# j-fu/ExtendableSparse.jl

Hardware: AMD Instinct MI355X
Metric: assembled+flushed nnz/sec and HBM GB/s %peak, 256³ 7-pt stencil, 1/2/4/8 GPU (higher is better)
Workload: dtype f64; 1 GPU; fdrand 256^3 Float64/Int64 fresh build: device COO append (the producer writes every update to its radix bucket) -> LDS bucket sort + ordered fold -> CSC (BASELINE.json configs[1]); n=256, appended_entries=200933376, final_nnz=117047296, partition=producer-side (append = partition), parallelism=1 GPU

## Files before the change

### extendablesparse.jl_amd/_lib.py

```python
import ctypes as C
import os

HERE = os.path.dirname(os.path.abspath(__file__))
SO = os.path.join(HERE, "libesparse_hip.so")

ESP_OK = 0
ESP_ERR_INVALID, ESP_ERR_BOUNDS, ESP_ERR_HIP, ESP_ERR_NOMEM = -1, -2, -3, -4
ESP_ERR_UNSUPPORTED, ESP_ERR_STATE, ESP_ERR_NODEVICE = -5, -6, -7
ESP_ERR_NOTPOSDEF = -8
ESP_SET, ESP_UPDATE, ESP_RAWUPDATE, ESP_COO = 0, 1, 2, 3
ESP_OP_ADD, ESP_OP_SUB = 0, 1
ESP_FLUSH_ROUTED, ESP_FLUSH_PLUS = 0, 1
ESP_PATH_NO_KEPT_STRUCTURE = 45
ESP_PRECON_JACOBI, ESP_PRECON_ILU0, ESP_PRECON_ILUAM, ESP_PRECON_BLOCK, ESP_PRECON_AMG = 0, 1, 2, 3, 4
ESP_PRECON_ILUK = 5
ESP_PRECON_COLORED = 6
ESP_PRECON_SPAI = 7
ESP_PRECON_ILUT = 8
ESP_PRECON_LU = 9
ESP_PRECON_CHOLESKY = 10
ESP_CHOL_STATS = 12
ESP_ILUT_WAVE_UPPER, ESP_ILUT_GROUP_UPPER, ESP_ILUT_STEPS_MAX, ESP_ILUT_STATS = 256, 4096, 16, 40
ESP_ILUK_WAVE_VISITS, ESP_ILUK_VISIT_MAX = 512, 8192
ESP_SPAI_WAVE_DOUBLES, ESP_SPAI_DENSE_MAX = 512, 12288
# ... 147 lines not shown
    "esp_transpose": (i32, [vp, vp, P(i64)]),
    "esp_debug_transpose_path": (i32, [vp, i32]),
    "esp_debug_last_transpose": (i32, [vp, P(i64)]),
    "esp_mul_transpose": (i32, [vp, vp, vp, i32]),
    "esp_issymmetric": (i32, [vp, P(i32)]),
    "esp_opnorm": (i32, [vp, f64, P(f64)]),
    "esp_norm": (i32, [vp, f64, P(f64)]),
    "esp_shard_counts": (i32, [vp, i32, vp]),
    "esp_shard_export": (i32, [vp, i32, vp, vp, vp]),
    "esp_shard_exchange_begin": (i32, [vp, i32, i32, i64, i64, P(vp), P(vp), vp]),
    "esp_shard_exchange_place": (i32, [vp, i64, vp, vp, i64]),
    "esp_shard_partition": (i32, [vp, i32, i32, i64, P(i32), P(vp), P(vp), P(vp), vp, P(i64)]),
    "esp_shard_assemble": (i32, [vp, vp, vp, vp, vp, P(i32)]),
    "esp_shard_plan": (i32, [vp, i32, i32, i64]),
    "esp_debug_last_shard_source": (i32, [vp, P(i32)]),
    "esp_debug_last_local_small": (i32, [vp, P(i32)]),
    "esp_debug_last_bucket_pairs": (i32, [vp, P(i32)]),
    "esp_debug_last_bucket_cut": (i32, [vp, P(i32), P(i32)]),
    "esp_debug_last_predicted": (i32, [vp, P(i32)]),
    "esp_debug_spoil_predicted": (i32, [vp]),
    "esp_debug_last_lazy_items": (i32, [vp, P(i32)]),
    "esp_debug_last_lazy_stencil": (i32, [vp, P(i32)]),
    "esp_debug_last_kept_structure": (i32, [vp, P(i32)]),
    "esp_debug_last_sum_join": (i32, [vp, P(i32)]),
    "esp_debug_last_sum_ms": (i32, [vp, P(C.c_double), P(C.c_double)]),
    "esp_debug_last_sum_batched": (i32, [vp, P(C.c_int32)]),
    "esp_debug_last_sum_plan_bits": (i32, [vp, P(i32), P(i32)]),
    "esp_debug_last_rebuild": (i32, [vp, P(i32)]),
    "esp_group_unique_id": (i32, [vp]),
    "esp_group_create": (i32, [vp, i32, i32, vp, P(vp)]),
    "esp_group_create_comm": (i32, [vp, i32, i32, vp, P(vp)]),
    "esp_group_destroy": (i32, [vp]),
    "esp_group_handle": (i32, [vp, P(vp)]),
    "esp_group_last_error": (C.c_char_p, [vp]),
    "esp_group_column_range": (i32, [vp, P(i64), P(i64)]),
    "esp_group_flush": (i32, [vp, i32, P(i64), P(i32)]),
    "esp_group_nnz": (i32, [vp, P(i64), P(i64)]),
    "esp_group_get_csc": (i32, [vp, vp, vp, vp]),
    "esp_group_last_exchange": (i32, [vp, P(i32), P(i64)]),
    "esp_debug_group_loopback": (i32, [vp, i32, P(i64)]),
    "esp_timing_enable": (i32, [vp, i32]),
    "esp_timing": (i32, [vp, P(esp_timing_t), i32]),
    "esp_debug_plan_cap": (i32, [vp, C.c_double]),
    "esp_debug_fail_next_bucket_stage": (i32, [vp]),
    "esp_debug_force_path": (i32, [vp, i32]),
    "esp_debug_last_run_order": (i32, [vp, P(i32)]),
# ... 49 lines not shown
```

### extendablesparse.jl_amd/csrc/flush.hip

```cpp
#include "internal.hpp"

bool esplocal::launch(const Variant &v, unsigned grid, hipStream_t stream, const Args &a) {
    if (v.pair) return launch_pair(v, grid, stream, a);
    if (v.g3) return launch_group3(v, grid, stream, a);
    if (v.grp) return v.shortg ? launch_group_short(v, grid, stream, a) : launch_group(v, grid, stream, a);
    if (v.pieces) return v.small_variant ? launch_pieces_small(v, grid, stream, a) : v.fresh ? launch_pieces_fresh(v, grid, stream, a) : launch_pieces_stored(v, grid, stream, a);
    return v.small_variant ? launch_small(v, grid, stream, a) : launch_regular(v, grid, stream, a);
}


int32_t finish_csc(esp_handle *h, i64 Z0, i64 Zn, const u64 *new_key, const double *new_val) {
    const i64 N1 = h->n + 1;
    u64 *colend = (u64 *)h->colend.p;
    i64 c0, ccnt;
    col_range(h, &c0, &ccnt);
    if (windowed(h)) h->tail_stale = h->wc1 < h->n;
    if (Z0 == 0) {
        Span sp(h, ESP_ST_COLPTR);
        sp.add(espscan::exclusive<u64, true>(h->stream, colend + c0, (u64 *)h->colptr.p + c0, ccnt, colend + N1, (u64)1));
        if (!windowed(h)) h->ones_pending = false;
        h->nnz = Zn;
        h->pattern_version++, h->values_version++;
        return ESP_OK;
    }
// ... 248 lines not shown
    return ESP_OK;
}

struct LocalTry {
    bool use_pred, want_wide, allow_g3;
    bool used_pair = false, used_g3 = false;
};

static int32_t launch_attempt(esp_handle *h, const Sorted &st, const LocalChoice &c, esplocal::Args &a, LocalTry &t) {
    Span sp(h, ESP_ST_LOCAL);
    const i64 max_grid = h->force_path == ESP_PATH_MANY_LAUNCHES ? 64 : esplocal::MAX_GRID;
    t.used_g3 = t.used_pair = false;
    if (c.pair_ok && !h->pair_off) {
        const int Sp = (c.S + 1) / 2;
        esplocal::Args ap = a;
        ap.S = Sp;
        ap.pair_buckets = c.S;
        ap.status = a.status + (c.S - Sp);
        esplocal::Variant var{true, false, false, true, c.pair_keys};
        var.pair = true;
        h->last_fold_update = c.pair_keys == 2 ? 1 : 0;
        const u64 out_cap = (u64)std::min(h->keys2.bytes / sizeof(i64), h->vals2.bytes / sizeof(double));
        const u64 *pred = (const u64 *)h->pred.tab.p;
        for (i64 first = 0; first < Sp; first += max_grid) {
            ap.first = first;
            const unsigned grid = (unsigned)std::min<i64>(max_grid, Sp - first);
            if (t.use_pred && st.stencil) {
                if (!esplocal::launch_pair_gen_predicted(var, grid, h->stream, ap, st.stencil->a, pred, out_cap, c.keep))
                    return ESP_RETRY_EXPANDED;
            } else if (!(t.use_pred ? esplocal::launch_pair_predicted(var, grid, h->stream, ap, pred, out_cap) : esplocal::launch(var, grid, h->stream, ap)))
                FAIL(h, ESP_ERR_STATE, "esp_flush: internal error (no pair kernel for this flush)");
        }
        t.used_pair = true;
        sp.add(1);
        return ESP_OK;
    }
    h->last_fold_update = (c.keys == 2 || c.keys == 3 || c.keys == 5 || c.keys == 7) ? 1 : 0;
    esplocal::Variant var{c.fresh, st.npieces > 0, c.big && !c.small_variant && !c.grp, c.small_variant, c.keys};
    var.shortg = c.grp && c.longest <= 32.0;
    var.grp = c.grp;
    var.g3 = t.allow_g3 && !h->g3_off && (c.g3_plain || (c.g3_k64 && !t.want_wide));
    var.g3k64 = var.g3 && c.g3_k64;
    if (var.g3k64) a.kind32 = (u32)c.kind_all;
    var.g3wide = var.g3 && t.want_wide;
    for (i64 first = 0; first < c.S; first += max_grid) {
        const unsigned grid = (unsigned)std::min<i64>(max_grid, c.S - first);
        a.first = first;
        t.used_g3 = var.g3;
        if (st.lazy) {
            if (!var.g3 || var.g3wide || !esplocal::launch_group3_items(*st.lazy, grid, h->stream, a)) return ESP_RETRY_EXPANDED;
        } else if (!esplocal::launch(var, grid, h->stream, a))
            FAIL(h, ESP_ERR_STATE, "esp_flush: internal error (no bucket kernel for this flush)");
    }
    sp.add(1);
    return ESP_OK;
// ... 87 lines not shown
    esplocal::Args a;
    fill_args(a, h, st, c, mode, lay);
    h->last_key_bytes = (st.p32_piece >= 0 || st.all32) ? 4 : st.key_bytes;
    const char *stamps_file = esp_exp_env("ESP_LOCAL_STAMPS");
    if (stamps_file) {
        CK(ensure(h, h->heads, sizeof(u64) * (size_t)c.S * 16));
        HIPCK(h, hipMemsetAsync(h->heads.p, 0, sizeof(u64) * (size_t)c.S * 16, h->stream));
        a.stamps = (unsigned long long *)h->heads.p;
    }
    LocalTry t{c.use_pred, c.want_wide, true};
    if (c.try_hits) {
        bool done = false;
        CK(try_hits_form(h, st, c, lay, a, t, Zn_out, &done));
        if (done) return ESP_OK;
    }
    CK(launch_attempt(h, st, c, a, t));
    CK(read_back(h, c, a));
    const bool pred_tried = t.use_pred && t.used_pair;
    if (pred_tried && (err_bits(h) & (esplocal::PRED_MISS | esplocal::PAIR_REFUSED))) {
        t.use_pred = false;
        h->pred.misses++;
        h->pred.last = 2;
        if (c.keep) h->last_kept = 2;
        drop_kept(h);
        CK(retry_attempt(h, st, c, lay, a, t));
    } else if (pred_tried) {
        h->pred.misses = 0;
        h->pred.last = 1;
    }
    if (t.used_pair && (err_bits(h) & esplocal::PAIR_REFUSED)) {
        h->pair_off = true;
        CK(retry_attempt(h, st, c, lay, a, t));
    }
    h->last_pair = t.used_pair ? 1 : 0;
    h->last_cl_bits = c.cl_bits;
    h->last_buckets = c.S;
    h->last_lazy_items = 0;
    h->last_sum_join = 0;
    if (st.lazy) {
        if (err_bits(h) & 8u) return ESP_RETRY_EXPANDED;
        h->last_lazy_items = 1;
    }
    if (t.used_g3 && !t.want_wide && h->force_path != ESP_PATH_NO_WIDE_GROUP3 && (err_bits(h) & (8u | 16u | 32u)) == (8u | 16u)) {
        t.want_wide = true;
        h->g3_wide = true;
        CK(retry_attempt(h, st, c, lay, a, t));
// ... 372 lines not shown
extern "C" int32_t esp_flush(esp_handle *h, int32_t mode, int64_t *new_nnz, int32_t *pattern_changed) {
    if (!h) return ESP_ERR_INVALID;
    if (mode != ESP_FLUSH_ROUTED && mode != ESP_FLUSH_PLUS) FAIL(h, ESP_ERR_INVALID, "esp_flush: mode");
    (void)hipSetDevice(h->device);
    if (pattern_changed) *pattern_changed = 0;
    i64 E = h->count;
    if (E == 0) {
        if (new_nnz) *new_nnz = h->nnz;
        return ESP_OK;
    }
    if (E >= 0xFFFFFFF0ll) FAIL(h, ESP_ERR_UNSUPPORTED, "esp_flush: %lld pending entries exceed the 2^32 limit of one flush", (long long)E);
    hipEvent_t fa = nullptr;
    if (h->timing) {
        fa = ev_get(h);
        (void)hipEventRecord(fa, h->stream);
    }
    i64 Zn = 0;
    h->last_rebuild = 0;
    h->last_pair = 0;
    h->pred.last = 0;
    h->kept.candidate = h->kept.valid;
    h->kept.valid = false;
    h->last_kept = 0;
    bool use_local = h->force_path != ESP_PATH_GENERAL;
    if (h->ones_pending && windowed(h)) CK(fix_tail(h));
    if (h->pre.valid) {
        const esp_handle::PrePart &pp = h->pre;
        const bool usable = use_local && !h->part_assembled && pp.mw_P == 0 && pp.E + pp.tail == E && pp.base == h->win_base &&
                            pp.span == h->win_span && pp.maxlen <= (i64)esplocal::CAP && pp.K - pp.pb <= esplocal::MAX_REM_BITS;
        if (!usable) CK(pending_materialize(h));
    }
    if (h->pre.valid && h->lazy.on &&
        (h->pre.tail != 0 || !use_local || windowed(h) || h->shard_user || h->part_assembled ||
         (h->nnz != 0 && !(h->seen_hits && !h->hits_off && mode == ESP_FLUSH_ROUTED))))
        CK(lazy_expand(h));
    if (h->pre.valid && h->lazyst.on &&
        (h->pre.tail != 0 || !use_local || windowed(h) || h->shard_user || h->part_assembled || h->nnz != 0))
        CK(lazy_expand(h));
    if (h->last_lazy_stencil == 1) h->last_lazy_stencil = 0;
    bool served = false, split = false, tail_direct = false;
    i64 Zsplit = 0;
    if (h->pre.valid && h->pre.tail > 0 && h->nnz > 0 && mode == ESP_FLUSH_ROUTED && h->force_path != ESP_PATH_BATCH_TAIL_ONE_FLUSH) {
        const esp_handle::PrePart pp = h->pre;
        Sorted st = pre_sorted(h, pp, false);
        st.expect_hits = 1;
        CK(ensure(h, h->keys2, sizeof(u64) * (size_t)E));
// ... 160 lines not shown
```

### extendablesparse.jl_amd/csrc/handle.hip

```cpp
#include "internal.hpp"

#include <pthread.h>
#include <sched.h>
#include <sys/mman.h>

#include <atomic>
#include <chrono>
#include <condition_variable>
#include <mutex>

thread_local std::string g_err;

int32_t ensure(esp_handle *h, DevBuf &b, size_t need, bool keep) {
    if (b.bytes >= need && b.p) return ESP_OK;
    if (h && (&b == &h->colptr || &b == &h->rowval || &b == &h->nzval)) drop_kept(h);
    size_t want = need;
    if (keep && b.bytes) want = std::max(need, b.bytes + b.bytes / 2);
    want = (want + 255) & ~(size_t)255;
    void *np = nullptr;
    if (!(keep && b.p && b.bytes)) {
        release(b);
        HIPCK(h, hipMalloc(&np, want));
        b.p = np;
        b.bytes = want;
// ... 199 lines not shown
    if (device < 0 || device >= ndev)
        FAIL((esp_handle *)nullptr, ESP_ERR_INVALID, "esp_create: device %d out of range (0..%d)", device, ndev - 1);
    const int rb = bits_for(m), cb = bits_for(n);
    if (rb + cb + ESP_TAG_BITS > 64)
        FAIL((esp_handle *)nullptr, ESP_ERR_UNSUPPORTED, "esp_create: %lld x %lld needs %d key bits (max 62)",
             (long long)m, (long long)n, rb + cb);
    esp_handle *h = new esp_handle();
    h->m = m;
    h->n = n;
    h->device = device;
    h->L = KeyLayout{rb, cb};
    h->win_base = 0;
    h->win_span = (u64)std::max<i64>(n, 1) << rb;
    h->wc0 = 0;
    h->wc1 = n;
    h->hint = capacity_hint > 0 ? capacity_hint : 0;
    memset(&h->acc, 0, sizeof h->acc);
    if (const char *e = getenv("ESP_DEBUG_FORCE_PATH")) h->force_path = atoi(e);
    if (hipSetDevice(device) != hipSuccess || hipStreamCreateWithFlags(&h->stream, hipStreamNonBlocking) != hipSuccess) {
        delete h;
        FAIL((esp_handle *)nullptr, ESP_ERR_HIP, "esp_create: cannot create a stream on device %d", device);
    }
    h->own_stream = true;
    if (hipHostMalloc((void **)&h->pin_scalar, 128, hipHostMallocDefault) != hipSuccess) {
        (void)hipStreamDestroy(h->stream);
        delete h;
        FAIL((esp_handle *)nullptr, ESP_ERR_NOMEM, "esp_create: pinned scalar allocation failed");
    }
    memset(h->pin_scalar, 0, 128);
    h->pin_words = h->pin_scalar + 8;
    if (hipHostGetDevicePointer((void **)&h->pin_words_dev, h->pin_words, 0) != hipSuccess || !h->pin_words_dev) {
        (void)hipHostFree(h->pin_scalar);
        (void)hipStreamDestroy(h->stream);
        delete h;
        FAIL((esp_handle *)nullptr, ESP_ERR_HIP, "esp_create: no device address for the pinned result words");
    }
    int32_t st = init_empty_csc(h);
    if (st == ESP_OK && capacity_hint > 0) {
        st = ensure(h, h->keys, sizeof(u64) * (size_t)capacity_hint);
        if (st == ESP_OK) st = ensure(h, h->vals, sizeof(double) * (size_t)capacity_hint);
        if (st == ESP_OK) h->cap = capacity_hint;
    }
    if (st != ESP_OK) {
        g_err = h->err;
        esp_destroy(h);
        return st;
// ... 1057 lines not shown
```

### extendablesparse.jl_amd/csrc/internal.hpp

```cpp
#pragma once
#include <stdio.h>
#include <stdlib.h>
#include <string.h>

#include <algorithm>
#include <functional>
#include <cmath>
#include <thread>

#include "common.hpp"
#include "fold.hpp"
#include "generators.hpp"
#include "femitems.hpp"
#include "elements.hpp"
#include "local_args.hpp"
#include "merge.hpp"
#include "radix.hpp"
#include "runpart.hpp"
#include "scan.hpp"


struct DevBuf {
    void *p = nullptr;
    size_t bytes = 0;
// ... 70 lines not shown
        espitem::Args it;
        espelem::Args el;
    } lazy;
    DevBuf lazy_hold;
    struct LazyStencil {
        bool on = false;
        bool armed = false;
        u64 gen = 0;
        unsigned grid = 0;
        espgen::FdArgs a;
    } lazyst;
    int last_lazy_stencil = 0;
    struct KeptStructure {
        bool valid = false;
        bool candidate = false;
        u64 plan_gen = 0, pred_gen = 0;
        i64 nx = 0, ny = 0, nz = 0;
        int keys = 0;
        const void *rowval = nullptr, *colptr = nullptr, *nzval = nullptr;
        i64 nnz = 0;
        unsigned long long pattern_version = 0;
    } kept;
    int last_kept = 0;
    int last_rebuild = 0;
    int last_lazy_items = 0;
    int last_sum_join = 0;
    int last_sum_plan_bits[2] = {0, 0};
    double last_sum_ms[2] = {0.0, 0.0};
    struct TailPart {
        bool valid = false;
        int K = 0, pb = 0;
        i64 T = 0, maxlen = 0;
        u64 base = 0, span = 0;
    } tailpart;
    struct RawPlan {
        bool valid = false;
        i64 count = 0, chunks = 0, maxlen = 0, maxlen_c = 0;
        int kind = 0, K = 0, pb = 0, key_bytes = 8, fb = 0;
        u64 base = 0, span = 0;
        double Ee = 0.0;
    } rawplan;
    struct PrePass {
        bool valid = false;
        i64 count = 0, maxlen = 0;
        int K = 0, planned = 0, npass = 0, bits0 = 0, cur = 0, S = 0;
        u64 base = 0, span = 0;
// ... 641 lines not shown
```

### extendablesparse.jl_amd/csrc/local_args.hpp

```cpp
#pragma once
#include "common.hpp"
#include "fold.hpp"

namespace espgen {
struct FdArgs;
}

namespace esplocal {

constexpr int THREADS = 512;
constexpr int WAVES = THREADS / ESP_WAVE;
constexpr int ITEMS = 8;
constexpr int CAP = THREADS * ITEMS;
constexpr int IDX_BITS = 12;
constexpr int SUB_SHIFT = ESP_TAG_BITS + IDX_BITS;
constexpr int MAX_REM_BITS = 64 - SUB_SHIFT;
static_assert((1 << IDX_BITS) == CAP, "slot index must cover the segment capacity");

constexpr int G3_CL_BITS = 8;
constexpr int CL_MAX_BITS = 11;
constexpr int CL_MAX = 1 << CL_MAX_BITS;
constexpr int REG_RUN = 24;
constexpr int REG_MAX_REM = 62 - SUB_SHIFT;
constexpr u64 NOREC = ~0ull;
// ... 28 lines not shown
    i64 total;
    i64 first;
    unsigned long long *stamps;
    int npieces;
    const i64 *pstart;
    const void *const *ptab;
    int pieces_dense;
    u32 *maxrun_seen;
    u32 kind32;
    int k32_piece;
    i64 k32_lo;
    i64 *colptr_out;
    i64 n_cols;
    i64 col_end;
    int late_total;
    int no_group;
    int kind_all;
    int expect_hits;
    int fb;
    const i64 *own_fine;
    double *hits_out;
    i64 pair_buckets;
    u64 *host_words;
};
constexpr int MAX_PIECES = 64;

struct MultiBuf {
    const u64 *sorted;
    const i64 *seg;
    const double *elmat;
    const char *cellrec;
    int negate;
    int low;
};
constexpr int MULTI_SEG_BITS = 20;

struct Variant {
    bool fresh;
    bool pieces;
    bool big;
    bool small_variant;
    int keys;
    bool grp = false;
    bool shortg = false;
    bool g3 = false;
    bool g3hits = false;
    bool g3wide = false;
    bool g3k64 = false;
    bool pair = false;
};
constexpr int PAIR_ITEMS = 12;
constexpr int PAIR_RUN = 12;
constexpr u32 PAIR_REFUSED = 128u;
constexpr u32 PRED_MISS = 256u;
bool launch(const Variant &v, unsigned grid, hipStream_t stream, const Args &a);
bool launch_regular(const Variant &v, unsigned grid, hipStream_t stream, const Args &a);
bool launch_small(const Variant &v, unsigned grid, hipStream_t stream, const Args &a);
bool launch_pieces_fresh(const Variant &v, unsigned grid, hipStream_t stream, const Args &a);
bool launch_pieces_stored(const Variant &v, unsigned grid, hipStream_t stream, const Args &a);
bool launch_pieces_small(const Variant &v, unsigned grid, hipStream_t stream, const Args &a);
bool launch_group(const Variant &v, unsigned grid, hipStream_t stream, const Args &a);
bool launch_group_short(const Variant &v, unsigned grid, hipStream_t stream, const Args &a);
bool launch_group3(const Variant &v, unsigned grid, hipStream_t stream, const Args &a);
bool launch_pair(const Variant &v, unsigned grid, hipStream_t stream, const Args &a);
bool launch_pair_predicted(const Variant &v, unsigned grid, hipStream_t stream, const Args &a, const u64 *pred, u64 out_cap);
bool launch_pair_gen_predicted(const Variant &v, unsigned grid, hipStream_t stream, const Args &a, const espgen::FdArgs &fd, const u64 *pred,
                               u64 out_cap, bool keep);
void launch_pair_record(hipStream_t stream, const i64 *colptr, i64 col_end, int ncl_bits, int Sp, u64 *pred);


}
```

### extendablesparse.jl_amd/csrc/local_x.hip

```cpp
#include "generators.hpp"
#include "local.hpp"
#include "pair.hpp"

namespace esplocal {

namespace {
constexpr int G_ROWS = 7;
constexpr int G_CAP = THREADS * G_ROWS;
}

struct StencilColumn {
    i64 stride[3];
    i64 i, j, k, nx, ny, nz;
    double vlo[3], vhi[3], vb[3];
    __device__ __forceinline__ bool lo(int q) const { return q == 0 ? k > 1 : q == 1 ? j > 1 : i > 1; }
    __device__ __forceinline__ bool hi(int q) const { return q == 0 ? i < nx : q == 1 ? j < ny : k < nz; }
    __device__ __forceinline__ bool b(int q) const {
        return q == 0 ? (i == 1 || i == nx) : q == 1 ? (ny > 2 && (j == 1 || j == ny)) : (nz > 2 && (k == 1 || k == nz));
    }
};

template <class F>
__device__ __forceinline__ double draw_if(bool on, F f) {
    return __ballot(on) != 0 ? f() : 0.0;
}

template <int MODE>
struct FdSource {
    static constexpr bool positive = MODE == 0 || MODE == 1;
    i64 nx, ny, nz;
    double hx, hy, hz;
    u64 seed;
    int fast;
    u64 magic_nx, magic_nxny;
    u64 zsub[3];

    struct Consts {
        espgen::SharedDiv x, y, z;
        __device__ __forceinline__ explicit Consts(const FdSource &s) : x(s.hx), y(s.hy), z(s.hz) {}
    };
    __device__ __forceinline__ double over(double n, const espgen::SharedDiv &by) const {
        return by.quot_mid(n);
    }
    __device__ __forceinline__ u64 z0(i64 g) const { return seed + (6ull * (u64)g + 1ull) * ESP_GOLDEN; }

    __device__ __forceinline__ void upper(const Consts &k, i64 g, StencilColumn &c) const {
        espgen::fd_node(*this, g, &c.i, &c.j, &c.k);
        constexpr int md = MODE;
        const u64 zg = z0(g);
        c.stride[0] = nx * ny, c.stride[1] = nx, c.stride[2] = 1;
        c.nx = nx, c.ny = ny, c.nz = nz;
        c.vhi[0] = over(espgen::fd_rand_z(md, zg, 0) * hy * hz, k.x);
        c.vhi[1] = over(espgen::fd_rand_z(md, zg, 2) * hx * hz, k.y);
        c.vhi[2] = over(espgen::fd_rand_z(md, zg, 4) * hx * hy, k.z);
    }
    __device__ __forceinline__ void lower(const Consts &k, i64 g, int t, const double *sx, const double *sy, StencilColumn &c) const {
        constexpr int md = MODE;
        const u64 zg = z0(g);
        const bool x_in = c.lo(2) && t >= 1, y_in = c.lo(1) && (i64)t >= nx;
        const double x_lds = sx[x_in ? t - 1 : 0], y_lds = sy[y_in ? t - (int)nx : 0];
        c.vlo[0] = draw_if(c.lo(0), [&] { return over(espgen::fd_rand_z(md, zg - zsub[0], 4) * hx * hy, k.z); });
        const double y_drawn = draw_if(c.lo(1) && !y_in, [&] { return over(espgen::fd_rand_z(md, zg - zsub[1], 2) * hx * hz, k.y); });
        const double x_drawn = draw_if(c.lo(2) && !x_in, [&] { return over(espgen::fd_rand_z(md, zg - zsub[2], 0) * hy * hz, k.x); });
        c.vlo[1] = y_in ? y_lds : y_drawn;
        c.vlo[2] = x_in ? x_lds : x_drawn;
        c.vb[0] = draw_if(c.b(0), [&] { return espgen::fd_rand_z(md, zg, 1) * hy * hz; });
        c.vb[1] = draw_if(c.b(1), [&] { return espgen::fd_rand_z(md, zg, 3) * hx * hz; });
        c.vb[2] = draw_if(c.b(2), [&] { return espgen::fd_rand_z(md, zg, 5) * hx * hy; });
    }
};

template <int KEYS, class SRC, bool KEEP>
__global__ __launch_bounds__(THREADS, 6) void pair_gen_pred_k(Args a, SRC src, const u64 *pred, u64 out_cap) {
    static_assert(KEYS == 1 || KEYS == 2, "one kind: 2 = every update is an UPDATE");
    constexpr bool UPD = KEYS == 2;
    constexpr bool FLAGS = UPD && SRC::positive;
    __shared__ u32 srow[KEEP ? 1 : G_CAP];
    __shared__ double sval[G_CAP];
    __shared__ double shx[THREADS], shy[THREADS];
    __shared__ u32 lw[WAVES];

    const int t = threadIdx.x, lane = t & 63, w = t >> 6;
    const int s = (int)(a.first + (i64)blockIdx.x);
    if (s >= a.S) return;
    const u64 dst = esp_uniform_u64(pred[s]);
    const u64 dst_next = esp_uniform_u64(pred[s + 1]);
    const int ncl = 2 << a.cl_bits;
    const u64 hi = ((u64)s << (a.rem_bits + 1)) + a.base;
    const i64 c_lo = (i64)(hi >> a.rb);
    const i64 c_hi = min(c_lo + (i64)ncl, a.col_end);
    const bool has = c_lo + t < c_hi;
    bool present[G_ROWS];
    double acc[G_ROWS];
    u32 row[G_ROWS];
#pragma unroll
    for (int q = 0; q < G_ROWS; q++) present[q] = false, acc[q] = 0.0, row[q] = 0u;
    const typename SRC::Consts k(src);
    StencilColumn c;
    if (has) {
        src.upper(k, c_lo + t, c);
        shx[t] = c.vhi[0];
        shy[t] = c.vhi[1];
    }
    __syncthreads();
    if (has) {
        src.lower(k, c_lo + t, t, shx, shy, c);
        const i64 l = c_lo + t + 1;
#pragma unroll
        for (int q = 0; q < 3; q++) row[q] = (u32)(l - c.stride[q]), row[4 + q] = (u32)(l + c.stride[2 - q]);
        row[3] = (u32)l;
        if constexpr (FLAGS) {
#pragma unroll
            for (int q = 0; q < 3; q++) {
                present[q] = c.lo(q), acc[q] = -c.vlo[q];
                present[4 + q] = c.hi(q), acc[4 + q] = -c.vhi[q];
            }
            bool any = false;
            double d = 0.0;
#pragma unroll
            for (int q = 0; q < 3; q++) any = any || c.lo(q), d = d + (c.lo(q) ? c.vlo[q] : 0.0);
#pragma unroll
            for (int q = 0; q < 3; q++) {
                any = any || c.hi(q) || c.b(q);
                d = d + (c.hi(q) ? c.vhi[q] : 0.0);
                d = d + (c.b(q) ? c.vb[q] : 0.0);
            }
            present[3] = any, acc[3] = d;
        } else {
            auto step = [&](int q, bool on, double v) {
                if (!on) return;
                if constexpr (UPD)
                    espfold::fold_step_update(present[q], acc[q], v);
                else
                    espfold::fold_step_sel(present[q], acc[q], a.kind32, v);
            };
#pragma unroll
            for (int q = 0; q < 3; q++) step(q, c.lo(q), -c.vlo[q]);
#pragma unroll
            for (int q = 0; q < 3; q++) step(3, c.lo(q), c.vlo[q]);
#pragma unroll
            for (int q = 0; q < 3; q++) {
                step(3, c.hi(q), c.vhi[q]);
                step(3, c.b(q), c.vb[q]);
            }
#pragma unroll
            for (int q = 0; q < 3; q++) step(4 + q, c.hi(q), -c.vhi[q]);
        }
    }
    u32 ec = 0;
#pragma unroll
    for (int q = 0; q < G_ROWS; q++) ec += present[q] ? 1u : 0u;
    const PairPlace pl = pair_place(ec, lw, lane, w);
    if (!pair_table_hit(dst, dst_next, pl.total, out_cap, s)) {
        if (t == 0) a.host_words[1] = (u64)PRED_MISS;
        return;
    }
    {
        u32 at = pl.at0;
#pragma unroll
        for (int q = 0; q < G_ROWS; q++) {
            if (present[q]) {
                if constexpr (!KEEP) srow[at] = row[q];
                sval[at] = acc[q];
                at++;
            }
        }
    }
    __syncthreads();
    pair_store<KEEP>(a, srow, sval, 0, dst, pl, hi, ncl, s, t);
    if (s == a.S - 1 && t == 0) a.host_words[0] = pair_grand_total(dst, pl.total);
}

bool launch_pair_gen_predicted(const Variant &v, unsigned grid, hipStream_t stream, const Args &a, const espgen::FdArgs &fd, const u64 *pred,
                               u64 out_cap, bool keep) {
    if (!v.fresh || v.pieces || a.cl_bits < 0 || (2 << a.cl_bits) > THREADS || a.rb >= 32 || !a.colptr_out || !a.host_words) return false;
    auto mid = [](double h) { return h >= 0x1.0p-100 && h <= 0x1.0p100; };
    if (!(mid(fd.hx) && mid(fd.hy) && mid(fd.hz))) return false;
    auto go = [&](auto M) {
        using Src = FdSource<decltype(M)::value>;
        const Src src{fd.nx, fd.ny, fd.nz, fd.hx, fd.hy, fd.hz, fd.seed, fd.fast, fd.magic_nx, fd.magic_nxny,
                      {6ull * (u64)(fd.nx * fd.ny) * ESP_GOLDEN, 6ull * (u64)fd.nx * ESP_GOLDEN, 6ull * ESP_GOLDEN}};
        return pair_for_keys(v.keys, [&](auto K) {
            constexpr int KEYS = decltype(K)::value;
            if (keep)
                hipLaunchKernelGGL((pair_gen_pred_k<KEYS, Src, true>), dim3(grid), dim3(THREADS), 0, stream, a, src, pred, out_cap);
            else
                hipLaunchKernelGGL((pair_gen_pred_k<KEYS, Src, false>), dim3(grid), dim3(THREADS), 0, stream, a, src, pred, out_cap);
        });
    };
    if (fd.rand_mode == 0) return go(std::integral_constant<int, 0>{});
    if (fd.rand_mode == 1) return go(std::integral_constant<int, 1>{});
    return go(std::integral_constant<int, 2>{});
}

}
```

### extendablesparse.jl_amd/csrc/shard.hip

```cpp
#include "internal.hpp"

int32_t shard_prepare(esp_handle *h, int P, espradix::Pass *out) {
    if (P < 1 || P > 256) FAIL(h, ESP_ERR_INVALID, "shards: nshards must be in 1..256");
    h->shard_user = true;
    drop_kept(h);
    CK(pending_materialize(h));
    h->part_valid = h->part_assembled = false;
    drop_gen_plan(h), drop_raw_plan(h);
    if ((double)h->n * (double)P >= 9.0e18) FAIL(h, ESP_ERR_UNSUPPORTED, "shards: n*nshards overflows");
    const i64 E = h->count;
    int bits = 1;
    while ((1 << bits) < P) bits++;
    const i64 T = std::max<i64>(1, ceil_div<i64>(E, espradix::TILE));
    CK(ensure(h, h->seg[0], sizeof(i64) * 4));
    CK(ensure(h, h->tilef[0], sizeof(u64) * (size_t)(4 + espscan::workspace_elems(4))));
    espradix::Pass p;
    p.keys_in = (const u64 *)h->keys.p;
    p.vals_in = (const double *)h->vals.p;
    p.keys_out = nullptr;
    p.vals_out = nullptr;
    p.seg_start = (const i64 *)h->seg[0].p;
    p.tile_first = (const i64 *)h->tilef[0].p;
    p.S = 1;
    p.shift = 0;
// ... 330 lines not shown
    h->shard_plan.P = nshards;
    h->shard_plan.me = self;
    h->shard_plan.eps = entries_per_shard;
    return ESP_OK;
}
extern "C" int32_t esp_debug_last_rebuild(const esp_handle *h, int32_t *on) {
    if (!h || !on) return ESP_ERR_INVALID;
    *on = h->last_rebuild;
    return ESP_OK;
}
extern "C" int32_t esp_debug_last_lazy_items(const esp_handle *h, int32_t *on) {
    if (!h || !on) return ESP_ERR_INVALID;
    *on = h->last_lazy_items;
    return ESP_OK;
}
extern "C" int32_t esp_debug_last_lazy_stencil(const esp_handle *h, int32_t *state) {
    if (!h || !state) return ESP_ERR_INVALID;
    *state = h->last_lazy_stencil;
    return ESP_OK;
}
extern "C" int32_t esp_debug_last_kept_structure(const esp_handle *h, int32_t *state) {
    if (!h || !state) return ESP_ERR_INVALID;
    *state = h->last_kept;
    return ESP_OK;
}
extern "C" int32_t esp_debug_last_sum_join(const esp_handle *h, int32_t *segments) {
    if (!h || !segments) return ESP_ERR_INVALID;
    *segments = h->last_sum_join;
    return ESP_OK;
}
extern "C" int32_t esp_debug_last_local_small(const esp_handle *h, int32_t *small) {
    if (!h || !small) return ESP_ERR_INVALID;
    *small = h->last_group3 == 4 ? 5 : h->last_group3 == 3 ? 4 : h->last_group3 == 2 ? 3 : h->last_group3 ? 2 : h->last_local_small;
    return ESP_OK;
}
extern "C" int32_t esp_debug_last_bucket_pairs(const esp_handle *h, int32_t *on) {
    if (!h || !on) return ESP_ERR_INVALID;
    *on = h->last_pair;
    return ESP_OK;
}
extern "C" int32_t esp_debug_last_bucket_cut(const esp_handle *h, int32_t *cl_bits, int32_t *buckets) {
    if (!h || !cl_bits || !buckets) return ESP_ERR_INVALID;
    *cl_bits = h->last_cl_bits;
    *buckets = h->last_buckets;
    return ESP_OK;
}
// ... 251 lines not shown
```

### extendablesparse.jl_amd/matrix.py

```python
import ctypes as C

import numpy as np

from . import _lib as L
from ._lib import (ESP_COO, ESP_ERR_INVALID, ESP_ERR_UNSUPPORTED, ESP_FLUSH_PLUS, ESP_FLUSH_ROUTED, ESP_OP_ADD, ESP_OP_SUB,
                   ESP_RAWUPDATE, ESP_SET, ESP_UPDATE, BoundsError, check)

_OPS = {"+": ESP_OP_ADD, "-": ESP_OP_SUB, ESP_OP_ADD: ESP_OP_ADD, ESP_OP_SUB: ESP_OP_SUB}
try:
    import operator as _operator
    _OPS[_operator.add] = ESP_OP_ADD
    _OPS[_operator.sub] = ESP_OP_SUB
except Exception:
    pass


def _op(op):
    try:
        return _OPS[op]
    except (KeyError, TypeError):
        raise NotImplementedError("op %r is not supported by the device buffer (only + and -); "
                                  "use the CPU SparseMatrixLNK path for it" % (op,))


# ... 761 lines not shown
    def debug_last_predicted(self):
        p = C.c_int32()
        self._d.ck(self._d.lib.esp_debug_last_predicted(self._d.h, C.byref(p)))
        return p.value

    def debug_spoil_predicted(self):
        self._d.ck(self._d.lib.esp_debug_spoil_predicted(self._d.h))

    def debug_last_lazy_items(self):
        p = C.c_int32()
        self._d.ck(self._d.lib.esp_debug_last_lazy_items(self._d.h, C.byref(p)))
        return p.value

    def debug_last_lazy_stencil(self):
        p = C.c_int32()
        self._d.ck(self._d.lib.esp_debug_last_lazy_stencil(self._d.h, C.byref(p)))
        return p.value

    def debug_last_kept_structure(self):
        p = C.c_int32()
        self._d.ck(self._d.lib.esp_debug_last_kept_structure(self._d.h, C.byref(p)))
        return p.value

    def debug_last_rebuild(self):
        p = C.c_int32()
        self._d.ck(self._d.lib.esp_debug_last_rebuild(self._d.h, C.byref(p)))
        return p.value

    def debug_last_shard_source(self):
        p = C.c_int32()
        self._d.ck(self._d.lib.esp_debug_last_shard_source(self._d.h, C.byref(p)))
        return p.value

    def debug_last_partition(self):
        p = C.c_int32()
        self._d.ck(self._d.lib.esp_debug_last_partition(self._d.h, C.byref(p)))
        return p.value

    def debug_last_plan_reused(self):
        k = C.c_int32()
        self._d.ck(self._d.lib.esp_debug_last_plan_reused(self._d.h, C.byref(k)))
        return k.value

    def debug_last_append_route(self):
        p = C.c_int32()
        self._d.ck(self._d.lib.esp_debug_last_append_route(self._d.h, C.byref(p)))
# ... 188 lines not shown
```

### include/esparse_hip.h

```cpp
#ifndef ESPARSE_HIP_H
#define ESPARSE_HIP_H
#include <stdint.h>
#ifdef __cplusplus
extern "C" {
#endif

typedef struct esp_handle esp_handle;

typedef enum {
    ESP_OK = 0,
    ESP_ERR_INVALID = -1,
    ESP_ERR_BOUNDS = -2,
    ESP_ERR_HIP = -3,
    ESP_ERR_NOMEM = -4,
    ESP_ERR_UNSUPPORTED = -5,
    ESP_ERR_STATE = -6,
    ESP_ERR_NODEVICE = -7,
    ESP_ERR_NOTPOSDEF = -8
} esp_status;

typedef enum { ESP_SET = 0, ESP_UPDATE = 1, ESP_RAWUPDATE = 2, ESP_COO = 3 } esp_kind;

typedef enum { ESP_OP_ADD = 0, ESP_OP_SUB = 1 } esp_op;

// ... 282 lines not shown
    ESP_PATH_NO_FINE_PARTITION = 41,
    ESP_PATH_NO_BUCKET_PAIRS = 42,
    ESP_PATH_NO_PREDICTED_OFFSETS = 43,
    ESP_PATH_NO_LAZY_STENCIL = 44,
    ESP_PATH_NO_KEPT_STRUCTURE = 45,
    ESP_PATH_NO_PLAN_REUSE = 31
} esp_debug_path;
int32_t esp_debug_force_path(esp_handle *h, int32_t path);
int32_t esp_debug_plan_cap(esp_handle *h, double cap);
int32_t esp_debug_fail_next_bucket_stage(esp_handle *h);
int32_t esp_debug_last_path(const esp_handle *h, int32_t *path);
int32_t esp_debug_last_run_order(const esp_handle *h, int32_t *kind);
int32_t esp_debug_last_colptr_direct(const esp_handle *h, int32_t *direct);
int32_t esp_debug_last_key_bytes(const esp_handle *h, int32_t *bytes);
int32_t esp_debug_last_fold_update(const esp_handle *h, int32_t *on);
int32_t esp_debug_last_local_small(const esp_handle *h, int32_t *small);
int32_t esp_debug_last_bucket_pairs(const esp_handle *h, int32_t *on);
int32_t esp_debug_last_bucket_cut(const esp_handle *h, int32_t *cl_bits, int32_t *buckets);
int32_t esp_debug_last_predicted(const esp_handle *h, int32_t *state);
int32_t esp_debug_spoil_predicted(esp_handle *h);
int32_t esp_debug_last_lazy_items(const esp_handle *h, int32_t *on);
int32_t esp_debug_last_lazy_stencil(const esp_handle *h, int32_t *state);
int32_t esp_debug_last_kept_structure(const esp_handle *h, int32_t *state);
int32_t esp_debug_last_sum_join(const esp_handle *h, int32_t *segments);
int32_t esp_debug_last_sum_ms(const esp_handle *h, double *folds_ms, double *combine_ms);
int32_t esp_debug_last_sum_batched(const esp_handle *h, int32_t *batched);
int32_t esp_debug_last_sum_plan_bits(const esp_handle *h, int32_t *pb_min, int32_t *pb_max);
int32_t esp_debug_last_rebuild(const esp_handle *h, int32_t *on);
int32_t esp_debug_last_plan_reused(const esp_handle *h, int32_t *reused);
int32_t esp_debug_last_partition(const esp_handle *h, int32_t *kind);
int32_t esp_debug_last_append_route(const esp_handle *h, int32_t *route);

#ifdef __cplusplus
}
#endif
#endif
```

Measured before the change: 573.4 billion nnz/s.

## March pair-gen workgroups through consecutive z-planes, reusing the lower-face draw

Measured after the change: 589.0 billion nnz/s, median of 6. 1.03x the previous value.

```diff
diff --git a/extendablesparse.jl_amd/_lib.py b/extendablesparse.jl_amd/_lib.py
--- a/extendablesparse.jl_amd/_lib.py
+++ b/extendablesparse.jl_amd/_lib.py
@@ -193,6 +193,9 @@
     "esp_debug_last_lazy_items": (i32, [vp, P(i32)]),
     "esp_debug_last_lazy_stencil": (i32, [vp, P(i32)]),
     "esp_debug_last_kept_structure": (i32, [vp, P(i32)]),
+    "esp_debug_last_march": (i32, [vp, P(i32)]),
+    "esp_debug_force_march": (i32, [vp, i32]),
+    "esp_debug_march_rule": (i32, [i64, i64, i64, i32, i32, P(i32)]),
     "esp_debug_last_sum_join": (i32, [vp, P(i32)]),
     "esp_debug_last_sum_ms": (i32, [vp, P(C.c_double), P(C.c_double)]),
     "esp_debug_last_sum_batched": (i32, [vp, P(C.c_int32)]),
diff --git a/extendablesparse.jl_amd/csrc/flush.hip b/extendablesparse.jl_amd/csrc/flush.hip
--- a/extendablesparse.jl_amd/csrc/flush.hip
+++ b/extendablesparse.jl_amd/csrc/flush.hip
@@ -294,15 +294,20 @@
         h->last_fold_update = c.pair_keys == 2 ? 1 : 0;
         const u64 out_cap = (u64)std::min(h->keys2.bytes / sizeof(i64), h->vals2.bytes / sizeof(double));
         const u64 *pred = (const u64 *)h->pred.tab.p;
-        for (i64 first = 0; first < Sp; first += max_grid) {
+        i64 units = Sp;
+        if (t.use_pred && st.stencil) {
+            units = esplocal::pair_gen_set_march(ap, st.stencil->a, h->compute_units, h->force_march);
+        }
+        for (i64 first = 0; first < units; first += max_grid) {
             ap.first = first;
-            const unsigned grid = (unsigned)std::min<i64>(max_grid, Sp - first);
+            const unsigned grid = (unsigned)std::min<i64>(max_grid, units - first);
             if (t.use_pred && st.stencil) {
                 if (!esplocal::launch_pair_gen_predicted(var, grid, h->stream, ap, st.stencil->a, pred, out_cap, c.keep))
                     return ESP_RETRY_EXPANDED;
             } else if (!(t.use_pred ? esplocal::launch_pair_predicted(var, grid, h->stream, ap, pred, out_cap) : esplocal::launch(var, grid, h->stream, ap)))
                 FAIL(h, ESP_ERR_STATE, "esp_flush: internal error (no pair kernel for this flush)");
         }
+        if (t.use_pred && st.stencil) h->last_march = ap.march;
         t.used_pair = true;
         sp.add(1);
         return ESP_OK;
@@ -436,6 +441,7 @@
         h->pred.misses++;
         h->pred.last = 2;
         if (c.keep) h->last_kept = 2;
+        h->last_march = 0;
         drop_kept(h);
         CK(retry_attempt(h, st, c, lay, a, t));
     } else if (pred_tried) {
@@ -854,6 +860,7 @@
     h->kept.candidate = h->kept.valid;
     h->kept.valid = false;
     h->last_kept = 0;
+    h->last_march = 0;
     bool use_local = h->force_path != ESP_PATH_GENERAL;
     if (h->ones_pending && windowed(h)) CK(fix_tail(h));
     if (h->pre.valid) {
diff --git a/extendablesparse.jl_amd/csrc/handle.hip b/extendablesparse.jl_amd/csrc/handle.hip
--- a/extendablesparse.jl_amd/csrc/handle.hip
+++ b/extendablesparse.jl_amd/csrc/handle.hip
@@ -245,6 +245,7 @@
         FAIL((esp_handle *)nullptr, ESP_ERR_HIP, "esp_create: cannot create a stream on device %d", device);
     }
     h->own_stream = true;
+    if (hipDeviceGetAttribute(&h->compute_units, hipDeviceAttributeMultiprocessorCount, device) != hipSuccess) h->compute_units = 0;
     if (hipHostMalloc((void **)&h->pin_scalar, 128, hipHostMallocDefault) != hipSuccess) {
         (void)hipStreamDestroy(h->stream);
         delete h;
diff --git a/extendablesparse.jl_amd/csrc/internal.hpp b/extendablesparse.jl_amd/csrc/internal.hpp
--- a/extendablesparse.jl_amd/csrc/internal.hpp
+++ b/extendablesparse.jl_amd/csrc/internal.hpp
@@ -116,6 +116,9 @@
         unsigned long long pattern_version = 0;
     } kept;
     int last_kept = 0;
+    int last_march = 0;
+    int force_march = 0;
+    int compute_units = 0;
     int last_rebuild = 0;
     int last_lazy_items = 0;
     int last_sum_join = 0;
diff --git a/extendablesparse.jl_amd/csrc/local_args.hpp b/extendablesparse.jl_amd/csrc/local_args.hpp
--- a/extendablesparse.jl_amd/csrc/local_args.hpp
+++ b/extendablesparse.jl_amd/csrc/local_args.hpp
@@ -74,6 +74,7 @@
     double *hits_out;
     i64 pair_buckets;
     u64 *host_words;
+    int march, march_step;
 };
 constexpr int MAX_PIECES = 64;
 
@@ -118,6 +119,8 @@
 bool launch_pair_predicted(const Variant &v, unsigned grid, hipStream_t stream, const Args &a, const u64 *pred, u64 out_cap);
 bool launch_pair_gen_predicted(const Variant &v, unsigned grid, hipStream_t stream, const Args &a, const espgen::FdArgs &fd, const u64 *pred,
                                u64 out_cap, bool keep);
+i64 pair_gen_set_march(Args &a, const espgen::FdArgs &fd, int compute_units, int force);
+int pair_gen_march_rule(i64 nx, i64 ny, i64 nz, int cl_bits, int compute_units);
 void launch_pair_record(hipStream_t stream, const i64 *colptr, i64 col_end, int ncl_bits, int Sp, u64 *pred);
 
 
diff --git a/extendablesparse.jl_amd/csrc/local_x.hip b/extendablesparse.jl_amd/csrc/local_x.hip
--- a/extendablesparse.jl_amd/csrc/local_x.hip
+++ b/extendablesparse.jl_amd/csrc/local_x.hip
@@ -11,7 +11,7 @@
 
 struct StencilColumn {
     i64 stride[3];
-    i64 i, j, k, nx, ny, nz;
+    u32 i, j, k, nx, ny, nz;
     double vlo[3], vhi[3], vb[3];
     __device__ __forceinline__ bool lo(int q) const { return q == 0 ? k > 1 : q == 1 ? j > 1 : i > 1; }
     __device__ __forceinline__ bool hi(int q) const { return q == 0 ? i < nx : q == 1 ? j < ny : k < nz; }
@@ -37,29 +37,45 @@
 
     struct Consts {
         espgen::SharedDiv x, y, z;
-        __device__ __forceinline__ explicit Consts(const FdSource &s) : x(s.hx), y(s.hy), z(s.hz) {}
+        __device__ __forceinline__ explicit Consts(const FdSource &s) : x(s.hx), y(s.hy), z(s.hz) {
+            x.r = uniform(x.r), y.r = uniform(y.r), z.r = uniform(z.r);
+        }
+        __device__ __forceinline__ static double uniform(double v) {
+            return __longlong_as_double((long long)esp_uniform_u64((u64)__double_as_longlong(v)));
+        }
     };
     __device__ __forceinline__ double over(double n, const espgen::SharedDiv &by) const {
         return by.quot_mid(n);
     }
     __device__ __forceinline__ u64 z0(i64 g) const { return seed + (6ull * (u64)g + 1ull) * ESP_GOLDEN; }
 
-    __device__ __forceinline__ void upper(const Consts &k, i64 g, StencilColumn &c) const {
-        espgen::fd_node(*this, g, &c.i, &c.j, &c.k);
+    __device__ __forceinline__ u64 begin(i64 g, StencilColumn &c) const {
+        i64 i, j, k;
+        espgen::fd_node(*this, g, &i, &j, &k);
+        c.i = (u32)i, c.j = (u32)j, c.k = (u32)k;
+        c.stride[0] = nx * ny, c.stride[1] = nx, c.stride[2] = 1;
+        c.nx = (u32)nx, c.ny = (u32)ny, c.nz = (u32)nz;
+        return z0(g);
+    }
+    __device__ __forceinline__ u64 next_plane(u64 zg, StencilColumn &c) const {
+        c.k += 1;
+        return zg + zsub[0];
+    }
+    __device__ __forceinline__ void upper(const Consts &k, u64 zg, StencilColumn &c) const {
         constexpr int md = MODE;
-        const u64 zg = z0(g);
-        c.stride[0] = nx * ny, c.stride[1] = nx, c.stride[2] = 1;
-        c.nx = nx, c.ny = ny, c.nz = nz;
         c.vhi[0] = over(espgen::fd_rand_z(md, zg, 0) * hy * hz, k.x);
         c.vhi[1] = over(espgen::fd_rand_z(md, zg, 2) * hx * hz, k.y);
         c.vhi[2] = over(espgen::fd_rand_z(md, zg, 4) * hx * hy, k.z);
     }
-    __device__ __forceinline__ void lower(const Consts &k, i64 g, int t, const double *sx, const double *sy, StencilColumn &c) const {
+    __device__ __forceinline__ void lower(const Consts &k, u64 zg, int t, const double *sx, const double *sy, bool first, double z_below,
+                                          StencilColumn &c) const {
         constexpr int md = MODE;
-        const u64 zg = z0(g);
         const bool x_in = c.lo(2) && t >= 1, y_in = c.lo(1) && (i64)t >= nx;
         const double x_lds = sx[x_in ? t - 1 : 0], y_lds = sy[y_in ? t - (int)nx : 0];
-        c.vlo[0] = draw_if(c.lo(0), [&] { return over(espgen::fd_rand_z(md, zg - zsub[0], 4) * hx * hy, k.z); });
+        if (first)
+            c.vlo[0] = draw_if(c.lo(0), [&] { return over(espgen::fd_rand_z(md, zg - zsub[0], 4) * hx * hy, k.z); });
+        else
+            c.vlo[0] = z_below;
         const double y_drawn = draw_if(c.lo(1) && !y_in, [&] { return over(espgen::fd_rand_z(md, zg - zsub[1], 2) * hx * hz, k.y); });
         const double x_drawn = draw_if(c.lo(2) && !x_in, [&] { return over(espgen::fd_rand_z(md, zg - zsub[2], 0) * hy * hz, k.x); });
         c.vlo[1] = y_in ? y_lds : y_drawn;
@@ -70,8 +86,8 @@
     }
 };
 
-template <int KEYS, class SRC, bool KEEP>
-__global__ __launch_bounds__(THREADS, 6) void pair_gen_pred_k(Args a, SRC src, const u64 *pred, u64 out_cap) {
+template <int KEYS, class SRC, bool KEEP, bool MARCH>
+__global__ __launch_bounds__(THREADS, KEEP && MARCH ? 8 : 6) void pair_gen_pred_k(Args a, SRC src, const u64 *__restrict__ pred, u64 out_cap) {
     static_assert(KEYS == 1 || KEYS == 2, "one kind: 2 = every update is an UPDATE");
     constexpr bool UPD = KEYS == 2;
     constexpr bool FLAGS = UPD && SRC::positive;
@@ -81,94 +97,147 @@
     __shared__ u32 lw[WAVES];
 
     const int t = threadIdx.x, lane = t & 63, w = t >> 6;
-    const int s = (int)(a.first + (i64)blockIdx.x);
+    const int ncl = 2 << a.cl_bits;
+    int s = (int)(a.first + (i64)blockIdx.x), s_step = 0;
+    if constexpr (MARCH) {
+        const u32 wg = (u32)s, P = (u32)a.march_step, chunk = wg / P;
+        s = esp_uniform_i32((int)(chunk * (u32)a.march * P + (wg - chunk * P)));
+        s_step = (int)P;
+    }
     if (s >= a.S) return;
-    const u64 dst = esp_uniform_u64(pred[s]);
-    const u64 dst_next = esp_uniform_u64(pred[s + 1]);
-    const int ncl = 2 << a.cl_bits;
-    const u64 hi = ((u64)s << (a.rem_bits + 1)) + a.base;
-    const i64 c_lo = (i64)(hi >> a.rb);
-    const i64 c_hi = min(c_lo + (i64)ncl, a.col_end);
-    const bool has = c_lo + t < c_hi;
-    bool present[G_ROWS];
-    double acc[G_ROWS];
-    u32 row[G_ROWS];
-#pragma unroll
-    for (int q = 0; q < G_ROWS; q++) present[q] = false, acc[q] = 0.0, row[q] = 0u;
     const typename SRC::Consts k(src);
     StencilColumn c;
-    if (has) {
-        src.upper(k, c_lo + t, c);
-        shx[t] = c.vhi[0];
-        shy[t] = c.vhi[1];
-    }
-    __syncthreads();
-    if (has) {
-        src.lower(k, c_lo + t, t, shx, shy, c);
-        const i64 l = c_lo + t + 1;
-#pragma unroll
-        for (int q = 0; q < 3; q++) row[q] = (u32)(l - c.stride[q]), row[4 + q] = (u32)(l + c.stride[2 - q]);
-        row[3] = (u32)l;
-        if constexpr (FLAGS) {
-#pragma unroll
-            for (int q = 0; q < 3; q++) {
-                present[q] = c.lo(q), acc[q] = -c.vlo[q];
-                present[4 + q] = c.hi(q), acc[4 + q] = -c.vhi[q];
+    const i64 g = (i64)((((u64)s << (a.rem_bits + 1)) + a.base) >> a.rb) + t;
+    const bool has = g < min(g - t + (i64)ncl, a.col_end);
+    u64 zg = 0ull;
+    if (has) zg = src.begin(g, c);
+    c.vhi[2] = 0.0;
+    u32 l = (u32)g + 1u;
+#pragma nounroll
+    for (int m = 0;;) {
+        const u64 dst = esp_uniform_u64(pred[s]);
+        const u64 dst_next = esp_uniform_u64(pred[s + 1]);
+        const u64 hi = ((u64)s << (a.rem_bits + 1)) + a.base;
+        bool present[G_ROWS];
+        double acc[G_ROWS];
+        u32 row[G_ROWS];
+#pragma unroll
+        for (int q = 0; q < G_ROWS; q++) present[q] = false, acc[q] = 0.0, row[q] = 0u;
+        const double z_below = c.vhi[2];
+        if (has) {
+            src.upper(k, zg, c);
+            shx[t] = c.vhi[0];
+            shy[t] = c.vhi[1];
+        }
+        __syncthreads();
+        if (has) {
+            src.lower(k, zg, t, shx, shy, m == 0, z_below, c);
+#pragma unroll
+            for (int q = 0; q < 3; q++) row[q] = l - (u32)c.stride[q], row[4 + q] = l + (u32)c.stride[2 - q];
+            row[3] = l;
+            if constexpr (FLAGS) {
+#pragma unroll
+                for (int q = 0; q < 3; q++) {
+                    present[q] = c.lo(q), acc[q] = -c.vlo[q];
+                    present[4 + q] = c.hi(q), acc[4 + q] = -c.vhi[q];
+                }
+                bool any = false;
+                double d = 0.0;
+#pragma unroll
+                for (int q = 0; q < 3; q++) any = any || c.lo(q), d = d + (c.lo(q) ? c.vlo[q] : 0.0);
+#pragma unroll
+                for (int q = 0; q < 3; q++) {
+                    any = any || c.hi(q) || c.b(q);
+                    d = d + (c.hi(q) ? c.vhi[q] : 0.0);
+                    d = d + (c.b(q) ? c.vb[q] : 0.0);
+                }
+                present[3] = any, acc[3] = d;
+            } else {
+                auto step = [&](int q, bool on, double v) {
+                    if (!on) return;
+                    if constexpr (UPD)
+                        espfold::fold_step_update(present[q], acc[q], v);
+                    else
+                        espfold::fold_step_sel(present[q], acc[q], a.kind32, v);
+                };
+#pragma unroll
+                for (int q = 0; q < 3; q++) step(q, c.lo(q), -c.vlo[q]);
+#pragma unroll
+                for (int q = 0; q < 3; q++) step(3, c.lo(q), c.vlo[q]);
+#pragma unroll
+                for (int q = 0; q < 3; q++) {
+                    step(3, c.hi(q), c.vhi[q]);
+                    step(3, c.b(q), c.vb[q]);
+                }
+#pragma unroll
+                for (int q = 0; q < 3; q++) step(4 + q, c.hi(q), -c.vhi[q]);
             }
-            bool any = false;
-            double d = 0.0;
-#pragma unroll
-            for (int q = 0; q < 3; q++) any = any || c.lo(q), d = d + (c.lo(q) ? c.vlo[q] : 0.0);
-#pragma unroll
-            for (int q = 0; q < 3; q++) {
-                any = any || c.hi(q) || c.b(q);
-                d = d + (c.hi(q) ? c.vhi[q] : 0.0);
-                d = d + (c.b(q) ? c.vb[q] : 0.0);
+        }
+        u32 ec = 0;
+#pragma unroll
+        for (int q = 0; q < G_ROWS; q++) ec += present[q] ? 1u : 0u;
+        const PairPlace pl = pair_place(ec, lw, lane, w);
+        if (!pair_table_hit(dst, dst_next, pl.total, out_cap, s)) {
+            if (t == 0) a.host_words[1] = (u64)PRED_MISS;
+            return;
+        }
+        {
+            u32 at = pl.at0;
+#pragma unroll
+            for (int q = 0; q < G_ROWS; q++) {
+                if (present[q]) {
+                    if constexpr (!KEEP) srow[at] = row[q];
+                    sval[at] = acc[q];
+                    at++;
+                }
             }
-            present[3] = any, acc[3] = d;
-        } else {
-            auto step = [&](int q, bool on, double v) {
-                if (!on) return;
-                if constexpr (UPD)
-                    espfold::fold_step_update(present[q], acc[q], v);
-                else
-                    espfold::fold_step_sel(present[q], acc[q], a.kind32, v);
-            };
-#pragma unroll
-            for (int q = 0; q < 3; q++) step(q, c.lo(q), -c.vlo[q]);
-#pragma unroll
-            for (int q = 0; q < 3; q++) step(3, c.lo(q), c.vlo[q]);
-#pragma unroll
-            for (int q = 0; q < 3; q++) {
-                step(3, c.hi(q), c.vhi[q]);
-                step(3, c.b(q), c.vb[q]);
-            }
-#pragma unroll
-            for (int q = 0; q < 3; q++) step(4 + q, c.hi(q), -c.vhi[q]);
-        }
-    }
-    u32 ec = 0;
-#pragma unroll
-    for (int q = 0; q < G_ROWS; q++) ec += present[q] ? 1u : 0u;
-    const PairPlace pl = pair_place(ec, lw, lane, w);
-    if (!pair_table_hit(dst, dst_next, pl.total, out_cap, s)) {
-        if (t == 0) a.host_words[1] = (u64)PRED_MISS;
-        return;
-    }
-    {
-        u32 at = pl.at0;
-#pragma unroll
-        for (int q = 0; q < G_ROWS; q++) {
-            if (present[q]) {
-                if constexpr (!KEEP) srow[at] = row[q];
-                sval[at] = acc[q];
-                at++;
-            }
-        }
-    }
-    __syncthreads();
-    pair_store<KEEP>(a, srow, sval, 0, dst, pl, hi, ncl, s, t);
-    if (s == a.S - 1 && t == 0) a.host_words[0] = pair_grand_total(dst, pl.total);
+        }
+        __syncthreads();
+        pair_store<KEEP>(a, srow, sval, 0, dst, pl, hi, ncl, s, t);
+        if (s == a.S - 1 && t == 0) a.host_words[0] = pair_grand_total(dst, pl.total);
+        if (!MARCH || ++m >= a.march) return;
+        s += s_step;
+        if (s >= a.S) return;
+        if (has) l += (u32)c.stride[0], zg = src.next_plane(zg, c);
+    }
+}
+
+namespace {
+constexpr int MARCH_PLANES = 3;
+constexpr i64 MARCH_RESIDENT_PER_CU = 4;
+constexpr i64 MARCH_ROUNDS_X4 = 43;
+i64 march_pairs_per_plane(i64 nx, i64 ny, int cl_bits) {
+    if (nx < 1 || ny < 1 || cl_bits < 0 || (2 << cl_bits) > THREADS) return 0;
+    const i64 ncl = (i64)2 << cl_bits, nxny = nx * ny;
+    return nxny % ncl == 0 ? nxny / ncl : 0;
+}
+}
+
+int pair_gen_march_rule(i64 nx, i64 ny, i64 nz, int cl_bits, int compute_units) {
+    const i64 P = march_pairs_per_plane(nx, ny, cl_bits);
+    if (P == 0 || nz < MARCH_PLANES) return 1;
+    const i64 R = MARCH_RESIDENT_PER_CU * (i64)std::max(compute_units, 1);
+    auto workgroups = [&](i64 L) { return P * ((nz + L - 1) / L); };
+    auto planes_per_slot = [&](i64 L) { return L * ((4 * workgroups(L) + R + 4 * R - 1) / (4 * R)); };
+    const i64 L = MARCH_PLANES;
+    return 4 * workgroups(L) >= MARCH_ROUNDS_X4 * R && planes_per_slot(L) * 32 <= planes_per_slot(1) * 33 ? (int)L : 1;
+}
+
+static int pair_gen_march(const Args &a, const espgen::FdArgs &fd, int compute_units, int force) {
+    const i64 P = march_pairs_per_plane(fd.nx, fd.ny, a.cl_bits);
+    if (P == 0 || fd.nz < 1 || a.rb >= 32 || (a.base >> a.rb) != 0 || a.col_end != fd.nx * fd.ny * fd.nz || (i64)a.S != P * fd.nz || P > 0x7fffffff)
+        return 1;
+    if (force > 0) return (int)std::min<i64>(force, fd.nz);
+    return pair_gen_march_rule(fd.nx, fd.ny, fd.nz, a.cl_bits, compute_units);
+}
+
+i64 pair_gen_set_march(Args &a, const espgen::FdArgs &fd, int compute_units, int force) {
+    a.march = pair_gen_march(a, fd, compute_units, force);
+    a.march_step = 0;
+    if (a.march <= 1) return (i64)a.S;
+    const i64 P = march_pairs_per_plane(fd.nx, fd.ny, a.cl_bits);
+    a.march_step = (int)P;
+    return P * ((fd.nz + a.march - 1) / a.march);
 }
 
 bool launch_pair_gen_predicted(const Variant &v, unsigned grid, hipStream_t stream, const Args &a, const espgen::FdArgs &fd, const u64 *pred,
@@ -176,16 +245,23 @@
     if (!v.fresh || v.pieces || a.cl_bits < 0 || (2 << a.cl_bits) > THREADS || a.rb >= 32 || !a.colptr_out || !a.host_words) return false;
     auto mid = [](double h) { return h >= 0x1.0p-100 && h <= 0x1.0p100; };
     if (!(mid(fd.hx) && mid(fd.hy) && mid(fd.hz))) return false;
+    if (a.march > 1 && (a.march != pair_gen_march(a, fd, 0, a.march) || (i64)a.march_step != march_pairs_per_plane(fd.nx, fd.ny, a.cl_bits)))
+        return false;
     auto go = [&](auto M) {
         using Src = FdSource<decltype(M)::value>;
         const Src src{fd.nx, fd.ny, fd.nz, fd.hx, fd.hy, fd.hz, fd.seed, fd.fast, fd.magic_nx, fd.magic_nxny,
                       {6ull * (u64)(fd.nx * fd.ny) * ESP_GOLDEN, 6ull * (u64)fd.nx * ESP_GOLDEN, 6ull * ESP_GOLDEN}};
         return pair_for_keys(v.keys, [&](auto K) {
             constexpr int KEYS = decltype(K)::value;
-            if (keep)
-                hipLaunchKernelGGL((pair_gen_pred_k<KEYS, Src, true>), dim3(grid), dim3(THREADS), 0, stream, a, src, pred, out_cap);
-            else
-                hipLaunchKernelGGL((pair_gen_pred_k<KEYS, Src, false>), dim3(grid), dim3(THREADS), 0, stream, a, src, pred, out_cap);
+            auto run = [&](auto KP, auto MA) {
+                hipLaunchKernelGGL((pair_gen_pred_k<KEYS, Src, decltype(KP)::value, decltype(MA)::value>), dim3(grid), dim3(THREADS), 0, stream, a,
+                                   src, pred, out_cap);
+            };
+            const bool march = a.march > 1;
+            if (keep && march) run(std::true_type{}, std::true_type{});
+            else if (keep) run(std::true_type{}, std::false_type{});
+            else if (march) run(std::false_type{}, std::true_type{});
+            else run(std::false_type{}, std::false_type{});
         });
     };
     if (fd.rand_mode == 0) return go(std::integral_constant<int, 0>{});
diff --git a/extendablesparse.jl_amd/csrc/shard.hip b/extendablesparse.jl_amd/csrc/shard.hip
--- a/extendablesparse.jl_amd/csrc/shard.hip
+++ b/extendablesparse.jl_amd/csrc/shard.hip
@@ -376,6 +376,21 @@
 extern "C" int32_t esp_debug_last_kept_structure(const esp_handle *h, int32_t *state) {
     if (!h || !state) return ESP_ERR_INVALID;
     *state = h->last_kept;
+    return ESP_OK;
+}
+extern "C" int32_t esp_debug_last_march(const esp_handle *h, int32_t *planes) {
+    if (!h || !planes) return ESP_ERR_INVALID;
+    *planes = h->last_march;
+    return ESP_OK;
+}
+extern "C" int32_t esp_debug_force_march(esp_handle *h, int32_t planes) {
+    if (!h || planes < 0) return ESP_ERR_INVALID;
+    h->force_march = planes;
+    return ESP_OK;
+}
+extern "C" int32_t esp_debug_march_rule(int64_t nx, int64_t ny, int64_t nz, int32_t cl_bits, int32_t compute_units, int32_t *planes) {
+    if (!planes || nx < 1 || ny < 1 || nz < 1) return ESP_ERR_INVALID;
+    *planes = esplocal::pair_gen_march_rule(nx, ny, nz, cl_bits, compute_units);
     return ESP_OK;
 }
 extern "C" int32_t esp_debug_last_sum_join(const esp_handle *h, int32_t *segments) {
diff --git a/extendablesparse.jl_amd/matrix.py b/extendablesparse.jl_amd/matrix.py
--- a/extendablesparse.jl_amd/matrix.py
+++ b/extendablesparse.jl_amd/matrix.py
@@ -807,6 +807,22 @@
         self._d.ck(self._d.lib.esp_debug_last_kept_structure(self._d.h, C.byref(p)))
         return p.value
 
+    def debug_last_march(self):
+        p = C.c_int32()
+        self._d.ck(self._d.lib.esp_debug_last_march(self._d.h, C.byref(p)))
+        return p.value
+
+    def debug_force_march(self, planes):
+        self._d.ck(self._d.lib.esp_debug_force_march(self._d.h, int(planes)))
+
+    @staticmethod
+    def debug_march_rule(nx, ny, nz, cl_bits, compute_units):
+        p = C.c_int32()
+        rc = L.load().esp_debug_march_rule(int(nx), int(ny), int(nz), int(cl_bits), int(compute_units), C.byref(p))
+        if rc != 0:
+            raise ValueError("esp_debug_march_rule: invalid arguments")
+        return p.value
+
     def debug_last_rebuild(self):
         p = C.c_int32()
         self._d.ck(self._d.lib.esp_debug_last_rebuild(self._d.h, C.byref(p)))
diff --git a/include/esparse_hip.h b/include/esparse_hip.h
--- a/include/esparse_hip.h
+++ b/include/esparse_hip.h
@@ -328,6 +328,9 @@
 int32_t esp_debug_last_lazy_items(const esp_handle *h, int32_t *on);
 int32_t esp_debug_last_lazy_stencil(const esp_handle *h, int32_t *state);
 int32_t esp_debug_last_kept_structure(const esp_handle *h, int32_t *state);
+int32_t esp_debug_last_march(const esp_handle *h, int32_t *planes);
+int32_t esp_debug_force_march(esp_handle *h, int32_t planes);
+int32_t esp_debug_march_rule(int64_t nx, int64_t ny, int64_t nz, int32_t cl_bits, int32_t compute_units, int32_t *planes);
 int32_t esp_debug_last_sum_join(const esp_handle *h, int32_t *segments);
 int32_t esp_debug_last_sum_ms(const esp_handle *h, double *folds_ms, double *combine_ms);
 int32_t esp_debug_last_sum_batched(const esp_handle *h, int32_t *batched);
```
